# maiziezhoulab/FocalSV

Measured on AMD Instinct MI355X. Metric: target regions/sec (50 kb, 30x HiFi), higher is better.
Workload: dtype u32; 1 GPU; 256 synthetic 50 kb regions per GPU, 30x HiFi-like reads U(10k,20k), 0.2% error, seed 1000+i (BASELINE.json configs[1]); regions_per_gpu=256

## Files before the change

focalsv_amd/csrc/k_sketch.h:

```cpp
#pragma once
#include "fsv_internal.h"

#define FSV_UQ_MAX     4096

namespace {

__device__ __forceinline__ uint64_t mix64(uint64_t key)
{
    key = ~key + (key << 21);
    key = key ^ key >> 24;
    key = (key + (key << 3)) + (key << 8);
    key = key ^ key >> 14;
    key = (key + (key << 2)) + (key << 4);
    key = key ^ key >> 28;
    key = key + (key << 31);
    return key;
}

__device__ __forceinline__ fsv_mz mz_make(uint64_t hash, uint32_t pos, uint32_t rev, uint32_t span)
{
    fsv_mz m; m.hash = hash; m.pos = pos; m.rev = (uint8_t)rev; m.span = (uint8_t)span; m.pad = 0;
    return m;
}
__device__ __forceinline__ void mz_pack(const fsv_mz m, uint64_t *hash, uint64_t *pay) { *hash = m.hash; *pay = (uint64_t)m.pos | (uint64_t)m.rev << 32 | (uint64_t)m.span << 40; }
__device__ __forceinline__ fsv_mz mz_unpack(uint64_t hash, uint64_t pay) { return mz_make(hash, (uint32_t)pay, (uint8_t)(pay >> 32), (uint8_t)(pay >> 40)); }

struct MzList { fsv_mz *out; uint32_t cap; uint32_t *cnt, *warn; };
__device__ __forceinline__ void mz_emit(const MzList &L, const fsv_mz rec)
{
    const uint32_t at = atomicAdd(L.cnt, 1u);
    if (at < L.cap) L.out[at] = rec;
    else atomicOr(L.warn, (uint32_t)FSV_W_MZ_TRUNC);
}

template <bool FLT> struct FltView { static constexpr bool on = false; };
template <> struct FltView<true> {
    static constexpr bool on = true;
    const unsigned long long *keys; const uint64_t *off; const uint32_t *read_set;
    __device__ __forceinline__ KmerSet set_of(uint32_t r) const { const uint32_t s = read_set[r]; const uint64_t base = off[s]; return KmerSet{base, off[s + 1] - base}; }
};
struct SketchFilter { const unsigned long long *keys = nullptr; const uint64_t *off = nullptr; const uint32_t *read_set = nullptr; };
template <class Fn> int with_filter(const SketchFilter &f, Fn fn) { return f.keys ? fn(FltView<true>{f.keys, f.off, f.read_set}) : fn(FltView<false>{}); }

template <bool FLT> __device__ __forceinline__ KmerSet flt_set_of(const FltView<FLT> &F, uint32_t r)
{
    if constexpr (FLT) return F.set_of(r); else return KmerSet{0, 0};
}
template <bool FLT> __device__ __forceinline__ bool flt_dummy(const FltView<FLT> &F, const KmerSet &S, uint64_t h)
{
    if constexpr (FLT) return S.size && S.has(F.keys, h); else return false;
}

__host__ __device__ inline size_t sketch_lds_bytes(int w, uint32_t read_words) { return (size_t)read_words * 4 + (size_t)w * 64 * 14 + 64 * 64 * 2 + 16; }

struct WordCache {
    const uint32_t *p; uint32_t w; int idx;
    __device__ __forceinline__ uint32_t get(int i) { const int wi = i >> 4; if (wi != idx) { w = p[wi]; idx = wi; } return (w >> ((i & 15) << 1)) & 3u; }
};

struct LaneDeque {
    uint64_t *hash;
    uint32_t *ps;
    uint16_t *tf;
    int w, head, cnt;
    __device__ __forceinline__ int slot(int j) const { const int x = head + j; return x >= w ? x - w : x; }
    __device__ __forceinline__ uint64_t hash_at(int sl) const { return hash[sl * 64]; }
    __device__ __forceinline__ uint64_t front() const { return hash[head * 64]; }
    __device__ __forceinline__ void expire(int tcur) { while (cnt > 0 && (((tcur - (int)(tf[head * 64] >> 2)) & 0x3fff) >= w)) { head = slot(1); cnt--; } }
    __device__ __forceinline__ void push(uint64_t h, uint32_t pos_span, int tcur, uint32_t rev)
    {
        while (cnt > 0 && hash_at(slot(cnt - 1)) > h) cnt--;
        const int sl = slot(cnt);
        hash[sl * 64] = h; ps[sl * 64] = pos_span; tf[sl * 64] = (uint16_t)((uint32_t)tcur << 2 | rev << 1);
        cnt++;
    }
    __device__ __forceinline__ int front_run() const { const uint64_t m = front(); int run = 1; while (run < cnt && hash_at(slot(run)) == m) run++; return run; }
    __device__ __forceinline__ bool emitted(int sl) const { return tf[sl * 64] & 1u; }
    __device__ __forceinline__ void mark(int sl) { tf[sl * 64] = (uint16_t)(tf[sl * 64] | 1u); }
    __device__ __forceinline__ fsv_mz record(int sl) const { const uint32_t p = ps[sl * 64]; return mz_make(hash[sl * 64], p >> 8, (tf[sl * 64] >> 1) & 1u, p & 0xffu); }
};

struct RunRing {
    uint16_t *q; int head, cnt, span;
    __device__ __forceinline__ int push(int run, int k)
    {
        const int rs = min(run, 256);
        q[((head + cnt++) & 63) * 64] = (uint16_t)rs;
        span += rs;
        if (cnt > k) { span -= q[head * 64]; head = (head + 1) & 63; cnt--; }
        return span;
    }
};

template <bool FLT>
__global__ __launch_bounds__(64) void k_sketch(const uint32_t *__restrict__ store, const uint32_t *__restrict__ word_off,
                                               const int32_t *__restrict__ read_len, const uint32_t *__restrict__ mz_off,
                                               fsv_mz *__restrict__ mz, uint32_t *__restrict__ mz_cnt, uint32_t n_reads, int w, int k,
                                               int hpc, uint32_t *__restrict__ warn, const uint8_t *__restrict__ w_per_read, int w_max,
                                               uint32_t lds_words, const FltView<FLT> F)
{
    extern __shared__ __attribute__((aligned(16))) uint8_t s_dyn[];
    const int lane = threadIdx.x;
    const uint32_t r = blockIdx.x;
    if (r >= n_reads) return;
    const uint32_t woff = word_off[r];
    const int len = read_len[r];
    const MzList L{mz + mz_off[r], mz_off[r + 1] - mz_off[r], &mz_cnt[r], &warn[r]};
    if (w_per_read) w = w_per_read[r];
    [[maybe_unused]] const KmerSet fset = flt_set_of(F, r);
    uint64_t *d_hash = (uint64_t *)s_dyn;
    uint32_t *s_words = (uint32_t *)(d_hash + (size_t)w_max * 64);
    uint32_t *d_ps = s_words + lds_words;
    uint16_t *d_tf = (uint16_t *)(d_ps + (size_t)w_max * 64);
    uint16_t *q_run = d_tf + (size_t)w_max * 64;
    const uint32_t nwords = ((uint32_t)len + 15u) >> 4;
    const bool staged = nwords <= lds_words;
    if (staged) for (uint32_t i = lane; i < nwords; i += 64) s_words[i] = store[woff + i];
    __syncthreads();
    WordCache B{staged ? (const uint32_t *)s_words : store + woff, 0u, -1};
    const bool single = (k & 1) == 0;
    const int c0 = single ? 0 : (int)((long long)len * lane / 64), c1 = single ? (lane == 0 ? len : 0) : (int)((long long)len * (lane + 1) / 64);
    if (c1 <= c0) return;
    int b0 = c0;
    if (hpc) {
        while (b0 > 0 && B.get(b0 - 1) == B.get(b0)) b0--;
        for (int n = 0; n < w + k + 4 && b0 > 0; n++) {
            b0--;
            const uint32_t c = B.get(b0);
            while (b0 > 0 && B.get(b0 - 1) == c) b0--;
        }
    } else {
        b0 = max(0, c0 - (w + k + 4));
    }
    const uint64_t NONE = ~0ull;
    const uint64_t mask = (1ull << k) - 1;
    uint64_t km0 = 0, km1 = 0, km2 = 0, km3 = 0;
    LaneDeque D{d_hash + lane, d_ps + lane, d_tf + lane, w, 0, 0};
    RunRing Q{q_run + lane, 0, 0, 0};
    int span = 0;
    int l = b0 > 0 ? w + k + 1 : 0;
    int tail = -1;
    auto emit_slot = [&](int sl) {
        const fsv_mz m = D.record(sl);
        if ((int)m.pos >= c0 && (int)m.pos < c1) mz_emit(L, m);
        D.mark(sl);
    };

    int i = b0;
    for (; i < len; i++) {
        if (i >= c1) { if (tail < 0) tail = w + 2; if (tail-- == 0) break; }
        const uint32_t c = B.get(i);
        uint64_t cur_h = NONE; uint32_t cur_ps = 0; uint32_t cur_rev = 0;
        if (hpc) {
            int run = 1;
            while (i + run < len && B.get(i + run) == c) run++;
            i += run - 1;
            span = Q.push(run, k);
        } else {
            span = l + 1 < k ? l + 1 : k;
        }
        km0 = (km0 << 1 | (uint64_t)(c & 1u)) & mask;
        km1 = (km1 << 1 | (uint64_t)(c >> 1)) & mask;
        km2 = km2 >> 1 | (uint64_t)(1u - (c & 1u)) << (k - 1);
        km3 = km3 >> 1 | (uint64_t)(1u - (c >> 1)) << (k - 1);
        if (km1 == km3) continue;
        const int z = km1 < km3 ? 0 : 1;
        ++l;
        if (l >= k && span < 256) {
            cur_h = z ? mix64(km2) + mix64(km3) : mix64(km0) + mix64(km1);
            cur_ps = ((uint32_t)i << 8) | (uint32_t)span;
            cur_rev = (uint32_t)z;
            if (flt_dummy(F, fset, cur_h)) { cur_h = NONE; cur_ps = 0; cur_rev = 0; }
        }
        const int tcur = l & 0x3fff;
        D.expire(tcur);
        if (l == w + k - 1 && D.cnt > 0 && D.front() != NONE) {
            const uint64_t m = D.front();
            const int run = D.front_run();
            for (int j = 0; j + 1 < run; j++) emit_slot(D.slot(j));
            if (cur_h <= m) D.mark(D.slot(run - 1));
        }
        D.push(cur_h, cur_ps, tcur, cur_rev);
        if (l >= w + k - 1) {
            const uint64_t m = D.front();
            if (m != NONE)
                for (int j = 0; j < D.cnt; j++) {
                    const int sl = D.slot(j);
                    if (D.hash_at(sl) != m) break;
                    if (!D.emitted(sl)) emit_slot(sl);
                }
        }
    }
    if (i >= len && l < w + k - 1 && D.cnt > 0 && D.front() != NONE) emit_slot(D.slot(D.front_run() - 1));
}

template <class View>
__device__ __forceinline__ void bitonic_lds(View v, const uint32_t np)
{
    for (uint32_t sz = 2; sz <= np; sz <<= 1)
        for (uint32_t st = sz >> 1; st > 0; st >>= 1) {
            for (uint32_t t = threadIdx.x; t < np / 2; t += 256) {
                const uint32_t i = ((t & ~(st - 1)) << 1) | (t & (st - 1)), j = i | st;
                const bool up = (i & sz) == 0;
                if (v.before(j, i) == up) v.swap(i, j);
            }
            __syncthreads();
        }
}
struct ByHashPos {
    uint64_t *hash, *pay;
    __device__ __forceinline__ bool before(uint32_t a, uint32_t b) const
    {
        const uint64_t ha = hash[a], hb = hash[b], pa = pay[a], pb = pay[b];
        return (ha < hb) | ((ha == hb) & ((uint32_t)pa < (uint32_t)pb));
    }
    __device__ __forceinline__ void swap(uint32_t a, uint32_t b) const { const uint64_t ha = hash[a], hb = hash[b], pa = pay[a], pb = pay[b]; hash[a] = hb; hash[b] = ha; pay[a] = pb; pay[b] = pa; }
};
struct ByPos {
    uint64_t *hash, *pay;
    __device__ __forceinline__ bool before(uint32_t a, uint32_t b) const
    {
        const uint64_t pa = pay[a], pb = pay[b];
        if (pb == ~0ull) return pa != ~0ull;
        if (pa == ~0ull) return false;
        return (uint32_t)pa < (uint32_t)pb || ((uint32_t)pa == (uint32_t)pb && pa < pb);
    }
    __device__ __forceinline__ void swap(uint32_t a, uint32_t b) const { ByHashPos{hash, pay}.swap(a, b); }
};

template <class HashAt>
__device__ __forceinline__ bool occurs_once(HashAt hash_at, uint32_t i, uint32_t n, uint32_t max_occ = 1u)
{
    const uint64_t h = hash_at(i);
    bool u = (i == 0 || hash_at(i - 1) != h) && (i + 1 >= n || hash_at(i + 1) != h);
    if (max_occ > 1u && !u) {
        uint32_t run = 1;
        for (uint32_t d = 1; d <= max_occ && i >= d && hash_at(i - d) == h; d++) run++;
        for (uint32_t d = 1; d <= max_occ && i + d < n && hash_at(i + d) == h; d++) run++;
        u = run <= max_occ;
    }
    return u;
}
__device__ __forceinline__ void uniq_totals(unsigned long long *total, uint32_t unique, uint32_t raw, uint32_t slot)
{
    atomicAdd(total, (unsigned long long)unique);
    atomicAdd(total + 3, (unsigned long long)raw);
    atomicAdd(total + 4, (unsigned long long)(slot - 64u));
}

template <int UQ_MAX>
__device__ __forceinline__ void uniq_read(const uint32_t r, fsv_mz *__restrict__ mz, const uint32_t *__restrict__ mz_off, uint32_t *__restrict__ mz_cnt,
                                          uint32_t *__restrict__ warn, const uint32_t *__restrict__ only_changed, uint32_t lo_cnt, uint32_t hi_cnt,
                                          unsigned long long *__restrict__ total, const uint32_t max_occ = 1u)
{
    __shared__ uint64_t s_hash[UQ_MAX];
    __shared__ uint64_t s_pay[UQ_MAX];
    __shared__ uint32_t s_w[4];
    const int tid = threadIdx.x;
    if (only_changed && !only_changed[r]) return;
    { const uint32_t raw = mz_cnt[r]; if (raw <= lo_cnt || raw > hi_cnt) return; }
    fsv_mz *a = mz + mz_off[r];
    const uint32_t slot_cap = mz_off[r + 1] - mz_off[r];
    uint32_t n = min(mz_cnt[r], slot_cap);
    const uint32_t n_raw = n;
    if (n > UQ_MAX) { if (tid == 0) atomicOr(&warn[r], (uint32_t)FSV_W_MZ_TRUNC); n = UQ_MAX; }
    uint32_t np = 1;
    while (np < n) np <<= 1;
    for (uint32_t i = tid; i < np; i += 256) {
        if (i < n) mz_pack(a[i], &s_hash[i], &s_pay[i]);
        else { s_hash[i] = ~0ull; s_pay[i] = ~0ull; }
    }
    __syncthreads();
    bitonic_lds(ByHashPos{s_hash, s_pay}, np);
    const uint32_t per = (n + 255) / 256;
    const uint32_t lo = min(n, tid * per), hi = min(n, lo + per);
    uint64_t kh[UQ_MAX / 256], kp[UQ_MAX / 256];
    uint32_t cnt = 0;
#pragma unroll
    for (uint32_t j = 0; j < UQ_MAX / 256; j++) {
        const uint32_t i = lo + j;
        if (i < hi && occurs_once([&](uint32_t x) { return s_hash[x]; }, i, n, max_occ)) { kh[cnt] = s_hash[i]; kp[cnt] = s_pay[i]; cnt++; }
    }
    uint32_t m;
    const uint32_t o0 = block_offset_256(cnt, s_w, &m);
    if (tid == 0) {
        mz_cnt[r] = m;
        if (total) uniq_totals(total, m, n_raw, slot_cap);
    }
#pragma unroll
    for (uint32_t j = 0; j < UQ_MAX / 256; j++)
        if (j < cnt) { s_hash[o0 + j] = kh[j]; s_pay[o0 + j] = kp[j]; }
    __syncthreads();
    for (uint32_t i = tid; i < m; i += 256) a[i] = mz_unpack(s_hash[i], s_pay[i]);
    if (2 * m <= slot_cap) {
        uint32_t mp = 1;
        while (mp < m) mp <<= 1;
        for (uint32_t i = m + tid; i < mp; i += 256) { s_hash[i] = ~0ull; s_pay[i] = ~0ull; }
        __syncthreads();
        bitonic_lds(ByPos{s_hash, s_pay}, mp);
        for (uint32_t i = tid; i < m; i += 256) a[m + i] = mz_unpack(s_hash[i], s_pay[i]);
    } else if (tid == 0) atomicOr(&warn[r], (uint32_t)FSV_W_INTERNAL);
}

template <int UQ_MAX>
__global__ __launch_bounds__(256) void k_uniq(fsv_mz *__restrict__ mz, const uint32_t *__restrict__ mz_off, uint32_t *__restrict__ mz_cnt,
                                              uint32_t *__restrict__ warn, const uint32_t *__restrict__ only_changed = nullptr,
                                              uint32_t lo_cnt = 0u, uint32_t hi_cnt = 0xffffffffu, unsigned long long *__restrict__ total = nullptr,
                                              uint32_t max_occ = 1u)
{
    uniq_read<UQ_MAX>(blockIdx.x, mz, mz_off, mz_cnt, warn, only_changed, lo_cnt, hi_cnt, total, max_occ);
}

template <int UQ_MAX>
__global__ __launch_bounds__(256) void k_uniq_walk(fsv_mz *__restrict__ mz, const uint32_t *__restrict__ mz_off, uint32_t *__restrict__ mz_cnt,
                                                   uint32_t *__restrict__ warn, const uint32_t *__restrict__ only_changed, uint32_t lo_cnt, uint32_t hi_cnt,
                                                   unsigned long long *__restrict__ total, uint32_t n_reads)
{
    for (uint32_t r = blockIdx.x; r < n_reads; r += gridDim.x) {
        uniq_read<UQ_MAX>(r, mz, mz_off, mz_cnt, warn, only_changed, lo_cnt, hi_cnt, total);
        __syncthreads();
    }
}

#define FSV_UQ_SEG 16
#define FSV_UQ_LONG_GRID 32

__device__ __forceinline__ uint64_t mz_hash(const uint4 e) { return (uint64_t)e.x | (uint64_t)e.y << 32; }
template <bool BY_POS> __device__ __forceinline__ bool mz_less(const uint4 a, const uint4 b)
{
    if (BY_POS) return a.z < b.z;
    const uint64_t ha = mz_hash(a), hb = mz_hash(b);
    return ha < hb || (ha == hb && a.z < b.z);
}
template <bool BY_POS> struct LongTile {
    uint4 *e;
    __device__ __forceinline__ bool before(uint32_t a, uint32_t b) const { return mz_less<BY_POS>(e[a], e[b]); }
    __device__ __forceinline__ void swap(uint32_t a, uint32_t b) const { const uint4 ea = e[a], eb = e[b]; e[a] = eb; e[b] = ea; }
};

template <bool BY_POS>
__device__ __forceinline__ uint4 *sort_long(uint4 *a, uint4 *b, const uint32_t n, uint4 *s_e)
{
    const uint32_t tid = threadIdx.x;
    for (uint32_t base = 0; base < n; base += FSV_UQ_MAX) {
        const uint32_t nt = min((uint32_t)FSV_UQ_MAX, n - base);
        uint32_t np = 1;
        while (np < nt) np <<= 1;
        for (uint32_t i = tid; i < np; i += 256) s_e[i] = i < nt ? a[base + i] : make_uint4(~0u, ~0u, ~0u, ~0u);
        __syncthreads();
        bitonic_lds(LongTile<BY_POS>{s_e}, np);
        for (uint32_t i = tid; i < nt; i += 256) a[base + i] = s_e[i];
        __syncthreads();
    }
    uint4 *src = a, *dst = b;
    for (uint32_t wd = FSV_UQ_MAX; wd < n; wd <<= 1) {
        __threadfence_block();
        __syncthreads();
        const uint32_t n_seg = (n + FSV_UQ_SEG - 1) / FSV_UQ_SEG;
        for (uint32_t g = tid; g < n_seg; g += 256) {
            const uint32_t o0 = g * FSV_UQ_SEG;
            const uint32_t lo = o0 & ~(2u * wd - 1u), mid = min(lo + wd, n), hi = min(lo + 2u * wd, n);
            const uint32_t nx = mid - lo, ny = hi - mid, d = o0 - lo;
            const uint4 *X = src + lo, *Y = src + mid;
            uint32_t il = d > ny ? d - ny : 0u, ih = min(d, nx);
            while (il < ih) { const uint32_t i = (il + ih) >> 1; if (mz_less<BY_POS>(X[i], Y[d - i - 1])) il = i + 1; else ih = i; }
            uint32_t i = il, j = d - il;
            const uint32_t o1 = min(o0 + (uint32_t)FSV_UQ_SEG, hi);
            bool hx = i < nx, hy = j < ny;
            uint4 x = make_uint4(0, 0, 0, 0), y = x;
            if (hx) x = X[i];
            if (hy) y = Y[j];
            for (uint32_t o = o0; o < o1; o++) {
                const bool tx = hx && (!hy || mz_less<BY_POS>(x, y));
                dst[o] = tx ? x : y;
                if (tx) { i++; hx = i < nx; if (hx) x = X[i]; }
                else { j++; hy = j < ny; if (hy) y = Y[j]; }
            }
        }
        uint4 *t = src; src = dst; dst = t;
    }
    __threadfence_block();
    __syncthreads();
    return src;
}

__global__ __launch_bounds__(256) void k_uniq_long(fsv_mz *mz, const uint32_t *__restrict__ mz_off, uint32_t *mz_cnt, uint32_t *__restrict__ warn,
                                                   const uint32_t *__restrict__ only_changed, unsigned long long *__restrict__ total, uint32_t n_reads,
                                                   uint4 *ws, uint32_t ws_stride, uint32_t *__restrict__ n_done)
{
    __shared__ uint4 s_e[FSV_UQ_MAX];
    __shared__ uint32_t s_w[4];
    const uint32_t tid = threadIdx.x;
    uint4 *const w0 = ws + (size_t)blockIdx.x * 2u * ws_stride, *const w1 = w0 + ws_stride;
    for (uint32_t r = blockIdx.x; r < n_reads; r += gridDim.x) {
        if (only_changed && !only_changed[r]) continue;
        const uint32_t cap = mz_off[r + 1] - mz_off[r];
        const uint32_t raw = mz_cnt[r];
        if (raw <= FSV_UQ_MAX) continue;
        const uint32_t n = min(raw, cap);
        if (n > ws_stride) { if (tid == 0) atomicOr(&warn[r], (uint32_t)FSV_W_INTERNAL); continue; }
        uint4 *const slot = (uint4 *)(mz + mz_off[r]);
        const uint4 *S = sort_long<false>(slot, w0, n, s_e);
        uint32_t m = 0;
        for (uint32_t base = 0; base < n; base += 256) {
            const uint32_t i = base + tid;
            const bool u = i < n && occurs_once([&](uint32_t x) { return mz_hash(S[x]); }, i, n);
            uint32_t all;
            const uint32_t at = block_rank_256(u, s_w, &all);
            if (u) w1[m + at] = S[i];
            m += all;
            __syncthreads();
        }
        __threadfence_block();
        __syncthreads();
        for (uint32_t i = tid; i < m; i += 256) slot[i] = w1[i];
        const uint4 *P = sort_long<true>(w1, w0, m, s_e);
        if (2u * m <= cap) for (uint32_t i = tid; i < m; i += 256) slot[m + i] = P[i];
        else if (tid == 0) atomicOr(&warn[r], (uint32_t)FSV_W_INTERNAL);
        if (tid == 0) {
            mz_cnt[r] = m;
            if (n_done) atomicAdd(n_done, 1u);
            if (total) uniq_totals(total, m, n, cap);
        }
        __syncthreads();
    }
}

#define SKF_T 1024
#define SKF_NW_MAX (SKF_T + 2 * 256)
#define SKF_V ((SKF_NW_MAX + 255) / 256)
#define SKF_NONE (~0ull)

template <bool FLT> struct HpcPlanes {
    uint32_t *ends;
    uint32_t *low, *high;
    int k; uint64_t kmask; int hpc;
    int M;
    FltView<FLT> F; KmerSet fset;
    __device__ __forceinline__ int span(int e) const { return hpc ? (int)ends[e] - (e - k >= 0 ? (int)ends[e - k] : -1) : k; }
    __device__ __forceinline__ uint64_t cut(const uint32_t *pl, int a) const
    {
        const int wd = a >> 5, sh = a & 31;
        const uint64_t lo64 = (uint64_t)pl[wd] | (uint64_t)pl[wd + 1] << 32;
        uint64_t v = lo64 >> sh;
        if (sh) v |= (uint64_t)pl[wd + 2] << (64 - sh);
        return v & kmask;
    }
    __device__ __forceinline__ uint64_t entry_hash(int e, int *z_out) const
    {
        if (e < k - 1 || e >= M) return SKF_NONE;
        if (span(e) >= 256) return SKF_NONE;
        const uint64_t lo = cut(low, e - k + 1), hi = cut(high, e - k + 1);
        const uint64_t f0 = __brevll(lo) >> (64 - k), f1 = __brevll(hi) >> (64 - k);
        const uint64_t r0 = ~lo & kmask, r1 = ~hi & kmask;
        const int z = f1 < r1 ? 0 : 1;
        if (z_out) *z_out = z;
        const uint64_t h = mix64(z ? r0 : f0) + mix64(z ? r1 : f1);
        if (flt_dummy(F, fset, h)) return SKF_NONE;
        return h;
    }
};

struct SkfTile {
    uint64_t h[SKF_NW_MAX];
    uint64_t wmin[SKF_NW_MAX];
    uint64_t am, ah;
    int abest, short_at;
    uint32_t scan[4];
};

template <bool FLT>
__device__ __forceinline__ void hpc_compress(HpcPlanes<FLT> &P, SkfTile &T, const uint32_t *__restrict__ words, const int len)
{
    const int tid = threadIdx.x;
    const int nwords = (len + 15) >> 4;
    uint32_t carry = 0;
    for (int wbase = 0; wbase < nwords; wbase += 256) {
        const int wi = wbase + tid;
        uint32_t flags = 0, word = 0;
        int nb = 0;
        if (wi < nwords) {
            word = words[wi];
            nb = min(16, len - wi * 16);
            if (P.hpc) {
                const uint32_t nextb = (wi + 1 < nwords) ? (words[wi + 1] & 3u) : 4u;
                const uint32_t shifted = (word >> 2) | (nextb << 30);
                uint32_t d = word ^ shifted;
                d = (d | (d >> 1)) & 0x55555555u;
                d = (d | (d >> 1)) & 0x33333333u; d = (d | (d >> 2)) & 0x0f0f0f0fu; d = (d | (d >> 4)) & 0x00ff00ffu; d = (d | (d >> 8)) & 0xffffu;
                flags = nb >= 16 ? d : (d & ((1u << nb) - 1u));
                if (len - 1 - wi * 16 < 16) flags |= 1u << (len - 1 - wi * 16);
            } else flags = nb >= 16 ? 0xffffu : ((1u << nb) - 1u);
        }
        const uint32_t cnt = __popc(flags);
        uint32_t trip_total;
        const uint32_t base = carry + block_offset_256(cnt, T.scan, &trip_total);
        if (cnt) {
            uint32_t lo = 0, hi = 0, rank = 0;
            for (int j = 0; j < nb; j++)
                if ((flags >> j) & 1u) {
                    const uint32_t b = (word >> (2 * j)) & 3u;
                    lo |= (b & 1u) << rank; hi |= (b >> 1) << rank;
                    P.ends[base + rank] = (uint32_t)(wi * 16 + j);
                    rank++;
                }
            const uint32_t wd = base >> 5, sh = base & 31u;
            atomicOr(&P.low[wd], lo << sh); atomicOr(&P.high[wd], hi << sh);
            if (sh + cnt > 32) { atomicOr(&P.low[wd + 1], lo >> (32 - sh)); atomicOr(&P.high[wd + 1], hi >> (32 - sh)); }
        }
        carry += trip_total;
        __syncthreads();
    }
    P.M = (int)carry;
    __threadfence_block();
    __syncthreads();
}

template <bool FLT>
__device__ __forceinline__ void stage_hashes(const HpcPlanes<FLT> &P, SkfTile &T, const int e0, const int NW)
{
    for (int idx = threadIdx.x; idx < NW; idx += 256) T.h[idx] = P.entry_hash(e0 + idx, nullptr);
    __syncthreads();
}

__device__ __forceinline__ void doubling_pass(SkfTile &T, uint64_t (&v)[SKF_V], const uint64_t *src, const int d, const bool is_max, const int NW)
{
    const int tid = threadIdx.x;
#pragma unroll
    for (int c = 0; c < SKF_V; c++) {
        const int i = tid + 256 * c;
        if (i < NW) {
            const uint64_t b = i + d < NW ? src[i + d] : (is_max ? 0ull : SKF_NONE);
            v[c] = is_max ? max(v[c], b) : min(v[c], b);
        }
    }
    __syncthreads();
#pragma unroll
    for (int c = 0; c < SKF_V; c++) { const int i = tid + 256 * c; if (i < NW) T.wmin[i] = v[c]; }
    __syncthreads();
}

__device__ __forceinline__ void window_minima(SkfTile &T, uint64_t (&v)[SKF_V], const int NW, const int w, const int p2)
{
    const int tid = threadIdx.x;
#pragma unroll
    for (int c = 0; c < SKF_V; c++) { const int i = tid + 256 * c; v[c] = i < NW ? T.h[i] : SKF_NONE; }
    if (w == 1) doubling_pass(T, v, T.h, 0, false, NW);
    else {
        doubling_pass(T, v, T.h, 1, false, NW);
        for (int d = 2; d < p2; d <<= 1) doubling_pass(T, v, T.wmin, d, false, NW);
        if (w > p2) doubling_pass(T, v, T.wmin, w - p2, false, NW);
    }
}

__device__ __forceinline__ void start_anomaly(SkfTile &T, const int M, const int T0, const int w, const int e0)
{
    if (threadIdx.x == 0) {
        T.short_at = -1; T.abest = -1; T.am = SKF_NONE; T.ah = SKF_NONE;
        if (M <= T0) {
            uint64_t m = SKF_NONE; int bp = -1;
            for (int p = max(0, M - w); p < M; p++) { const uint64_t h = T.h[p - e0]; if (h != SKF_NONE && h <= m) { m = h; bp = p; } }
            T.short_at = bp;
        } else {
            uint64_t m = SKF_NONE; int bp = -1;
            for (int p = T0 - w + 1; p <= T0 - 1; p++) { const uint64_t h = T.h[p - e0]; if (h != SKF_NONE && h <= m) { m = h; bp = p; } }
            T.am = m; T.abest = bp; T.ah = T.h[T0 - e0];
        }
    }
}

template <bool FLT>
__device__ __forceinline__ void report(const HpcPlanes<FLT> &P, SkfTile &T, uint64_t (&v)[SKF_V], const MzList &L, const int t0, const int T0, const int NW,
                                       const int w, const int p2)
{
    const int tid = threadIdx.x, M = P.M;
    if (M > T0) {
#pragma unroll
        for (int c = 0; c < SKF_V; c++) {
            const int i = tid + 256 * c, t = t0 + i;
            if (i < NW && !(t >= T0 && t <= M - 1 && i < SKF_T + w - 1)) { T.wmin[i] = 0ull; v[c] = 0ull; }
        }
        __syncthreads();
        if (w > 1) {
            for (int d = 1; d < p2; d <<= 1) doubling_pass(T, v, T.wmin, d, true, NW);
            if (w > p2) doubling_pass(T, v, T.wmin, w - p2, true, NW);
        }
    }
    for (int pi = tid; pi < SKF_T; pi += 256) {
        const int p = t0 + pi;
        if (p >= M) break;
        const uint64_t hp = T.h[pi + (w - 1)];
        if (hp == SKF_NONE) continue;
        bool e;
        if (M <= T0) e = (p == T.short_at);
        else {
            e = (p + w - 1 >= T0) && T.wmin[pi] == hp;
            if (p >= T0 - w + 1 && p <= T0 - 1 && T.am != SKF_NONE && hp == T.am) e = (p != T.abest) ? true : (T.ah > T.am);
        }
        if (e) {
            int z = 0;
            const uint64_t h = P.entry_hash(p, &z);
            mz_emit(L, mz_make(h, P.ends[p], (uint32_t)z, (uint32_t)P.span(p)));
        }
    }
    __syncthreads();
}

template <bool FLT>
__global__ __launch_bounds__(256) void k_sketch_fast(const uint32_t *__restrict__ store, const uint32_t *__restrict__ word_off,
                                                     const int32_t *__restrict__ read_len, const uint32_t *__restrict__ mz_off,
                                                     fsv_mz *__restrict__ mz, uint32_t *__restrict__ mz_cnt, uint32_t n_reads, int w, int k,
                                                     int hpc, uint32_t *__restrict__ warn, const uint8_t *__restrict__ w_per_read,
                                                     uint32_t *__restrict__ sc_ends, uint32_t *__restrict__ sc_low, uint32_t *__restrict__ sc_high,
                                                     const uint32_t *__restrict__ only_changed, const FltView<FLT> F)
{
    __shared__ SkfTile T;
    const uint32_t r = blockIdx.x;
    if (r >= n_reads) return;
    if (only_changed && !only_changed[r]) return;
    const uint32_t woff = word_off[r];
    const MzList L{mz + mz_off[r], mz_off[r + 1] - mz_off[r], &mz_cnt[r], &warn[r]};
    if (w_per_read) w = w_per_read[r];
    if (threadIdx.x == 0) mz_cnt[r] = 0;
    HpcPlanes<FLT> P{sc_ends + (size_t)woff * 16, sc_low + woff + r, sc_high + woff + r, k, (1ull << k) - 1, hpc, 0, F, flt_set_of(F, r)};
    hpc_compress(P, T, store + woff, read_len[r]);
    const int T0 = w + k - 2;
    const int NW = SKF_T + 2 * (w - 1);
    int p2 = 1;
    while (p2 * 2 <= w) p2 <<= 1;
    for (int t0 = 0; t0 < P.M; t0 += SKF_T) {
        const int e0 = t0 - (w - 1);
        stage_hashes(P, T, e0, NW);
        uint64_t v[SKF_V];
        window_minima(T, v, NW, w, p2);
        if (t0 == 0) start_anomaly(T, P.M, T0, w, e0);
        __syncthreads();
        report(P, T, v, L, t0, T0, NW, w, p2);
    }
}

struct SketchJob {
    const uint32_t *store; uint32_t n_reads; size_t total_words; uint32_t max_words;
    int w, k, hpc; const uint8_t *wper; int w_max;
    bool replay;
    const uint32_t *only_changed;
    SketchFilter flt = {};
};
template <class Ws> int launch_sketch(fsv_ctx *ctx, Ws &W, const SketchJob &J)
{
    const bool fast = (J.k & 1) && !J.replay;
    if (!(fast && J.only_changed)) TRY(zero(ctx, W.mz_cnt, J.n_reads));
    if (fast) {
        const size_t plane = J.total_words + J.n_reads + 8;
        TRY(ensure(ctx, W.sk_ends, J.total_words * 16 + 64));
        TRY(ensure_each(ctx, plane, W.sk_low, W.sk_high));
        TRY(zero(ctx, W.sk_low, plane));
        TRY(zero(ctx, W.sk_high, plane));
        return with_filter(J.flt, [&](auto F) -> int {
            FSV_LAUNCH(ctx, ctx->stream, k_sketch_fast<decltype(F)::on>, dim3(J.n_reads), dim3(256), 0, J.store, W.word_off.p, W.len.p, W.mz_off.p, W.mz.p,
                       W.mz_cnt.p, J.n_reads, J.w, J.k, J.hpc, W.warn.p, J.wper, W.sk_ends.p, W.sk_low.p, W.sk_high.p, J.only_changed, F);
            return FSV_OK;
        });
    }
    const uint32_t lds_words = J.max_words < 8192u ? J.max_words : 8192u;
    const size_t lds = sketch_lds_bytes(J.w_max, lds_words);
    return with_filter(J.flt, [&](auto F) -> int {
        FSV_HIP(ctx, hipFuncSetAttribute((const void *)k_sketch<decltype(F)::on>, hipFuncAttributeMaxDynamicSharedMemorySize, (int)lds));
        FSV_LAUNCH(ctx, ctx->stream, k_sketch<decltype(F)::on>, dim3(J.n_reads), dim3(64), lds, J.store, W.word_off.p, W.len.p, W.mz_off.p, W.mz.p, W.mz_cnt.p,
                   J.n_reads, J.w, J.k, J.hpc, W.warn.p, J.wper, J.w_max, lds_words, F);
        return FSV_OK;
    });
}

struct UniqJob {
    uint32_t n_reads, max_words;
    const uint32_t *only_changed;
    unsigned long long *total;
    bool full_lists; uint32_t max_slot, n_long;
    uint32_t *n_long_done;
};
template <class Ws, class F> int launch_uniq(fsv_ctx *ctx, Ws &W, const UniqJob &J, F before_long)
{
    FSV_LAUNCH(ctx, ctx->stream, k_uniq<1024>, dim3(J.n_reads), dim3(256), 0, W.mz.p, W.mz_off.p, W.mz_cnt.p, W.warn.p, J.only_changed, 0u, 1024u, J.total);
    if (J.max_words * 16u > 1024u)
        FSV_LAUNCH(ctx, ctx->stream, k_uniq_walk<FSV_UQ_MAX>, dim3(std::min<uint32_t>(J.n_reads, 2u * (uint32_t)ctx->n_cu)), dim3(256), 0, W.mz.p, W.mz_off.p,
                   W.mz_cnt.p, W.warn.p, J.only_changed, 1024u, J.full_lists ? (uint32_t)FSV_UQ_MAX : 0xffffffffu, J.total, J.n_reads);
    if (J.full_lists && J.max_words * 16u > (uint32_t)FSV_UQ_MAX && J.n_long) {
        const uint32_t grid = std::min<uint32_t>(J.n_long, FSV_UQ_LONG_GRID);
        TRY(ensure(ctx, W.uq_ws, (size_t)grid * 2u * J.max_slot));
        before_long();
        FSV_LAUNCH(ctx, ctx->stream, k_uniq_long, dim3(grid), dim3(256), 0, W.mz.p, W.mz_off.p, W.mz_cnt.p, W.warn.p, J.only_changed, J.total, J.n_reads,
                   W.uq_ws.p, J.max_slot, J.n_long_done);
    }
    return FSV_OK;
}

}
```

Before: 2522 regions/s.

## Stage run ends and bit planes in shared memory for sketch hashing

```diff
diff --git a/focalsv_amd/csrc/k_sketch.h b/focalsv_amd/csrc/k_sketch.h
--- a/focalsv_amd/csrc/k_sketch.h
+++ b/focalsv_amd/csrc/k_sketch.h
@@ -430,6 +430,9 @@
 #define SKF_NW_MAX (SKF_T + 2 * 256)
 #define SKF_V ((SKF_NW_MAX + 255) / 256)
 #define SKF_NONE (~0ull)
+#define SKF_ENDS_MAX (SKF_NW_MAX + 63)
+#define SKF_E ((SKF_ENDS_MAX + 255) / 256)
+#define SKF_PW 64
 
 template <bool FLT> struct HpcPlanes {
     uint32_t *ends;
@@ -437,28 +440,7 @@
     int k; uint64_t kmask; int hpc;
     int M;
     FltView<FLT> F; KmerSet fset;
-    __device__ __forceinline__ int span(int e) const { return hpc ? (int)ends[e] - (e - k >= 0 ? (int)ends[e - k] : -1) : k; }
-    __device__ __forceinline__ uint64_t cut(const uint32_t *pl, int a) const
-    {
-        const int wd = a >> 5, sh = a & 31;
-        const uint64_t lo64 = (uint64_t)pl[wd] | (uint64_t)pl[wd + 1] << 32;
-        uint64_t v = lo64 >> sh;
-        if (sh) v |= (uint64_t)pl[wd + 2] << (64 - sh);
-        return v & kmask;
-    }
-    __device__ __forceinline__ uint64_t entry_hash(int e, int *z_out) const
-    {
-        if (e < k - 1 || e >= M) return SKF_NONE;
-        if (span(e) >= 256) return SKF_NONE;
-        const uint64_t lo = cut(low, e - k + 1), hi = cut(high, e - k + 1);
-        const uint64_t f0 = __brevll(lo) >> (64 - k), f1 = __brevll(hi) >> (64 - k);
-        const uint64_t r0 = ~lo & kmask, r1 = ~hi & kmask;
-        const int z = f1 < r1 ? 0 : 1;
-        if (z_out) *z_out = z;
-        const uint64_t h = mix64(z ? r0 : f0) + mix64(z ? r1 : f1);
-        if (flt_dummy(F, fset, h)) return SKF_NONE;
-        return h;
-    }
+    int pl_last;
 };
 
 struct SkfTile {
@@ -481,9 +463,10 @@
         int nb = 0;
         if (wi < nwords) {
             word = words[wi];
+            const uint32_t next = words[min(wi + 1, nwords - 1)];
             nb = min(16, len - wi * 16);
             if (P.hpc) {
-                const uint32_t nextb = (wi + 1 < nwords) ? (words[wi + 1] & 3u) : 4u;
+                const uint32_t nextb = (wi + 1 < nwords) ? (next & 3u) : 4u;
                 const uint32_t shifted = (word >> 2) | (nextb << 30);
                 uint32_t d = word ^ shifted;
                 d = (d | (d >> 1)) & 0x55555555u;
@@ -516,10 +499,59 @@
     __syncthreads();
 }
 
+struct SkfRegs { uint32_t end[SKF_V], sz[SKF_V]; };
+
+__device__ __forceinline__ uint64_t cut_bits(const uint32_t *pl, const int a, const uint64_t kmask)
+{
+    const int wd = a >> 5;
+    const uint32_t sh = (uint32_t)a & 31u, x0 = pl[wd], x1 = pl[wd + 1], x2 = pl[wd + 2];
+    return ((uint64_t)__funnelshift_r(x0, x1, sh) | (uint64_t)__funnelshift_r(x1, x2, sh) << 32) & kmask;
+}
+
 template <bool FLT>
-__device__ __forceinline__ void stage_hashes(const HpcPlanes<FLT> &P, SkfTile &T, const int e0, const int NW)
-{
-    for (int idx = threadIdx.x; idx < NW; idx += 256) T.h[idx] = P.entry_hash(e0 + idx, nullptr);
+__device__ __forceinline__ void stage_hashes(const HpcPlanes<FLT> &P, SkfTile &T, uint64_t (&v)[SKF_V], SkfRegs &R, const int e0, const int NW)
+{
+    static_assert((SKF_ENDS_MAX + 2 * SKF_PW) * sizeof(uint32_t) <= sizeof(T.wmin), "the largest staged slice -- SKF_NW_MAX + 63 run ends and two planes -- has to fit in the tile it borrows");
+    const int tid = threadIdx.x, k = P.k;
+    uint32_t *s_ends = (uint32_t *)T.wmin, *s_pl = s_ends + SKF_ENDS_MAX;
+    const int NE = P.hpc ? NW + k : 0;
+    const int w0 = max(0, e0 - k + 1) >> 5;
+    uint32_t le[SKF_E], lp = 0;
+#pragma unroll
+    for (int c = 0; c < SKF_E; c++) le[c] = 256 * c < NE ? P.ends[min(max(e0 - k + tid + 256 * c, 0), P.M - 1)] : 0u;
+    if (tid < 2 * SKF_PW) lp = (tid < SKF_PW ? P.low : P.high)[min(w0 + (tid & (SKF_PW - 1)), P.pl_last)];
+#pragma unroll
+    for (int c = 0; c < SKF_E; c++) { const int j = tid + 256 * c; if (j < NE) s_ends[j] = le[c]; }
+    if (tid < 2 * SKF_PW) s_pl[tid] = lp;
+    __syncthreads();
+#pragma unroll
+    for (int c = 0; c < SKF_V; c++) {
+        const int i = tid + 256 * c, e = e0 + i;
+        uint64_t h = SKF_NONE;
+        uint32_t end = 0, sz = 0;
+        if (i < NW && e >= k - 1 && e < P.M) {
+            int span = k;
+            end = (uint32_t)e;
+            if (P.hpc) { end = s_ends[i + k]; span = (int)end - (e - k >= 0 ? (int)s_ends[i] : -1); }
+            if (span < 256) {
+                const int a = e - k + 1 - 32 * w0;
+                const uint64_t lo = cut_bits(s_pl, a, P.kmask), hi = cut_bits(s_pl + SKF_PW, a, P.kmask);
+                const uint64_t f0 = __brevll(lo) >> (64 - k), f1 = __brevll(hi) >> (64 - k);
+                const uint64_t r0 = ~lo & P.kmask, r1 = ~hi & P.kmask;
+                const int z = f1 < r1 ? 0 : 1;
+                h = mix64(z ? r0 : f0) + mix64(z ? r1 : f1);
+                sz = (uint32_t)span | (uint32_t)z << 8;
+            }
+        }
+        v[c] = h; R.end[c] = end; R.sz[c] = sz;
+    }
+#pragma unroll
+    for (int c = 0; c < SKF_V; c++) { const int i = tid + 256 * c; if (i < NW) T.h[i] = v[c]; }
+    if constexpr (FLT) {
+        for (int i = tid; i < NW; i += 256) { const uint64_t h = T.h[i]; if (h != SKF_NONE && flt_dummy(P.F, P.fset, h)) T.h[i] = SKF_NONE; }
+#pragma unroll
+        for (int c = 0; c < SKF_V; c++) { const int i = tid + 256 * c; if (i < NW) v[c] = T.h[i]; }
+    }
     __syncthreads();
 }
 
@@ -542,9 +574,6 @@
 
 __device__ __forceinline__ void window_minima(SkfTile &T, uint64_t (&v)[SKF_V], const int NW, const int w, const int p2)
 {
-    const int tid = threadIdx.x;
-#pragma unroll
-    for (int c = 0; c < SKF_V; c++) { const int i = tid + 256 * c; v[c] = i < NW ? T.h[i] : SKF_NONE; }
     if (w == 1) doubling_pass(T, v, T.h, 0, false, NW);
     else {
         doubling_pass(T, v, T.h, 1, false, NW);
@@ -569,11 +598,10 @@
     }
 }
 
-template <bool FLT>
-__device__ __forceinline__ void report(const HpcPlanes<FLT> &P, SkfTile &T, uint64_t (&v)[SKF_V], const MzList &L, const int t0, const int T0, const int NW,
-                                       const int w, const int p2)
-{
-    const int tid = threadIdx.x, M = P.M;
+__device__ __forceinline__ void report(SkfTile &T, uint64_t (&v)[SKF_V], const SkfRegs &R, const MzList &L, const int M, const int t0, const int T0,
+                                       const int NW, const int w, const int p2)
+{
+    const int tid = threadIdx.x;
     if (M > T0) {
 #pragma unroll
         for (int c = 0; c < SKF_V; c++) {
@@ -586,10 +614,11 @@
             if (w > p2) doubling_pass(T, v, T.wmin, w - p2, true, NW);
         }
     }
-    for (int pi = tid; pi < SKF_T; pi += 256) {
-        const int p = t0 + pi;
-        if (p >= M) break;
-        const uint64_t hp = T.h[pi + (w - 1)];
+#pragma unroll
+    for (int c = 0; c < SKF_V; c++) {
+        const int i = tid + 256 * c, pi = i - (w - 1), p = t0 + pi;
+        if (pi < 0 || pi >= SKF_T || p >= M) continue;
+        const uint64_t hp = T.h[i];
         if (hp == SKF_NONE) continue;
         bool e;
         if (M <= T0) e = (p == T.short_at);
@@ -597,11 +626,7 @@
             e = (p + w - 1 >= T0) && T.wmin[pi] == hp;
             if (p >= T0 - w + 1 && p <= T0 - 1 && T.am != SKF_NONE && hp == T.am) e = (p != T.abest) ? true : (T.ah > T.am);
         }
-        if (e) {
-            int z = 0;
-            const uint64_t h = P.entry_hash(p, &z);
-            mz_emit(L, mz_make(h, P.ends[p], (uint32_t)z, (uint32_t)P.span(p)));
-        }
+        if (e) mz_emit(L, mz_make(hp, R.end[c], R.sz[c] >> 8, R.sz[c] & 0xffu));
     }
     __syncthreads();
 }
@@ -619,23 +644,25 @@
     if (r >= n_reads) return;
     if (only_changed && !only_changed[r]) return;
     const uint32_t woff = word_off[r];
+    const int len = read_len[r];
     const MzList L{mz + mz_off[r], mz_off[r + 1] - mz_off[r], &mz_cnt[r], &warn[r]};
     if (w_per_read) w = w_per_read[r];
     if (threadIdx.x == 0) mz_cnt[r] = 0;
-    HpcPlanes<FLT> P{sc_ends + (size_t)woff * 16, sc_low + woff + r, sc_high + woff + r, k, (1ull << k) - 1, hpc, 0, F, flt_set_of(F, r)};
-    hpc_compress(P, T, store + woff, read_len[r]);
+    HpcPlanes<FLT> P{sc_ends + (size_t)woff * 16, sc_low + woff + r, sc_high + woff + r, k, (1ull << k) - 1, hpc, 0, F, flt_set_of(F, r), (len + 15) >> 4};
+    hpc_compress(P, T, store + woff, len);
     const int T0 = w + k - 2;
     const int NW = SKF_T + 2 * (w - 1);
     int p2 = 1;
     while (p2 * 2 <= w) p2 <<= 1;
     for (int t0 = 0; t0 < P.M; t0 += SKF_T) {
         const int e0 = t0 - (w - 1);
-        stage_hashes(P, T, e0, NW);
         uint64_t v[SKF_V];
+        SkfRegs R;
+        stage_hashes(P, T, v, R, e0, NW);
         window_minima(T, v, NW, w, p2);
         if (t0 == 0) start_anomaly(T, P.M, T0, w, e0);
         __syncthreads();
-        report(P, T, v, L, t0, T0, NW, w, p2);
+        report(T, v, R, L, P.M, t0, T0, NW, w, p2);
     }
 }
 
```

Measured after the change: 2171 regions/s. 0.861x the previous value.
